# sisl/Crux.jl

Hardware: AMD Instinct MI355X
Metric: env-steps/sec + grad-steps/sec, PPO 2048x32 rollout (higher is better)
Workload: dtype f32

## Files before the change

### crux.jl_amd/csrc/train_fs2.hip

```cpp
#include "train_fs2_kernel.h"

template <int IN, int OUT, int KIND, int ACT, int H2, int ACT2, bool TIMING, bool PX = false, bool PXK = false, bool LAG = false>
static int32_t launch_fs2_form(crux_ctx* c, TrainArgs& a, hipStream_t stream) {
  using Lt = Fs2LayoutFor<IN, OUT, H2, LAG, PX>;
  constexpr size_t lds = sizeof(float) * (size_t)(PX && Lt::BK_FITS ? Lt::TOTAL_BK : Lt::TOTAL);
  { const int32_t rc = crux_lds_attr_once<k_train_fs2<IN, OUT, KIND, ACT, H2, ACT2, TIMING, PX, PXK, LAG>>(c, lds); if (rc) return rc; }
  hipLaunchKernelGGL((k_train_fs2<IN, OUT, KIND, ACT, H2, ACT2, TIMING, PX, PXK, LAG>), dim3(32), dim3(512), lds, stream, a);
  return crux_launch_check(c, PXK ? "k_train_fs2 (replica group, periodic form)" : PX ? "k_train_fs2 (replica group)" : LAG ? "k_train_fs2 (lagrange_ppo_loss)" : "k_train_fs2");
}
template <int IN, int OUT, int KIND, int ACT, int H2, int ACT2, unsigned FORMS>
static int32_t launch_fs2_row(crux_ctx* c, TrainArgs a, hipStream_t stream) {
  const int which = stream == c->stream ? 0 : 1;
  constexpr size_t xfloats = (size_t)CRUX_XBUF_FLOATS;
  if (!c->xbuf[which]) { if (hipMalloc(&c->xbuf[which], sizeof(float) * xfloats + 256) != hipSuccess) return crux_fail(c, CRUX_ENOMEM, "learner exchange buffer"); }
  a.xbuf = (float*)c->xbuf[which]; a.xctr = (unsigned*)((char*)c->xbuf[which] + sizeof(float) * xfloats);
  HIPCHK(c, hipMemsetAsync(c->xbuf[which], 0, sizeof(float) * xfloats + 256, stream));
  a.xcd = which;
  if constexpr ((FORMS & LF_FS2_LAG) != 0) { if (a.lag) return launch_fs2_form<IN, OUT, KIND, ACT, H2, ACT2, false, false, false, true>(c, a, stream); }
  if (crux_grouped(c) && a.need_px) {
    a.px_hist = c->peer_hist ? 1 : 0; a.px_n = c->peer_n; a.px_rank = c->peer_rank; a.px_tab = c->peer_tab + which * CRUX_PX_MAXR;
    if (a.px_every > 1) return launch_fs2_form<IN, OUT, KIND, ACT, H2, ACT2, false, true, true>(c, a, stream);
    return launch_fs2_form<IN, OUT, KIND, ACT, H2, ACT2, false, true, false>(c, a, stream);
  }
  if constexpr ((FORMS & LF_FS2_TIMING) != 0) if (crux_sw().mfma_timing) {
    a.dbg = mf_timing_buf(c);
    if (!a.dbg) return crux_fail(c, CRUX_ENOMEM, "timing buffer");
    int32_t rc = launch_fs2_form<IN, OUT, KIND, ACT, H2, ACT2, true>(c, a, stream); if (rc) return rc;
    static const char* const nc[16] = {"loop", "wait staged", "fwdL1+T1", "fwdL2", "L3+pair barrier+head", "dW3+dZ2+stats+T2", "wait B_1", "dW2+send+dH1", "dZ1+db+dW1", "B_2+reduce+granules", "wait P1",
                                       "W2 loads+granule poll", "drain loads", "totals+adam W2+ssq", "adam small", "B_b+report+exit"};
    static const char* const nh[16] = {"loop", "fetch", "stage next", "wait B_1", "dW2+send+drain", "arrival 1+wait(leader)", "-", "-", "-", "wait B_2+reduce+granules", "wait P1",
                                       "W2 loads+granule poll", "drain loads", "totals+adam W2+ssq", "adam small", "B_b+exit"};
    MfTimingRow rows[12];
    for (int i = 0; i < 12; ++i) { const int wg = i / 3, w = i % 3 == 0 ? 0 : i % 3 == 1 ? 4 : 7; rows[i].row = 8 * wg + w; rows[i].names = w == 0 ? nc : nh;
      snprintf(rows[i].label, sizeof rows[i].label, "[fs2-timing] %d-%d wg %d %s wave %d:", IN, OUT, wg, w == 0 ? "compute" : "helper", w); }
    return mf_timing_dump(c, stream, rows, 12);
  }
  return launch_fs2_form<IN, OUT, KIND, ACT, H2, ACT2, false>(c, a, stream);
}

int32_t crux_launch_fs2(crux_ctx* c, const TrainArgs& a, const LearnerShape* row, hipStream_t stream) {
#define FS2_ROW(I, O, K, A1, H, A2, F) if constexpr (((F) & LF_FS2_BUILT) != 0) if (row->is(I, O, K, A1, H, A2)) return launch_fs2_row<I, O, K, A1, H, A2, (F)>(c, a, stream);
  CRUX_LEARNER_SHAPES(FS2_ROW)
#undef FS2_ROW
  return crux_fail(c, CRUX_EINVAL, "k_train_fs2: no instantiation for this shape");
}
```

### crux.jl_amd/csrc/train_fs2_kernel.h

```cpp
#pragma once
#include <type_traits>
#include "train_args.h"

#include "mfma_helpers.h"
#include "learner_shared.h"
#include "peer_wait.h"

#define FS_LD 72
#ifndef CRUX_FS2_LATE_PARTS
#define CRUX_FS2_LATE_PARTS 3
#endif
__device__ __forceinline__ int fs_tx(int q) { return (4 - q) & 3; }

template <int IN, int OUT, int NWG, bool HELP = false, int H2 = 64, bool LAG = false>
struct FsLayout {
  static_assert(H2 == 64 || H2 == 32, "second hidden layer: 64 or 32 units");
  static constexpr int MH = H2 / 32, NT2 = H2 / 16, HH = H2 / 2, W2N = H2 * MF_HID;
  static constexpr int NWC = 16 / NWG, TILES = NWC / 2;
  static constexpr int NW = HELP ? 2 * NWC : NWC, NT = 64 * NW;
  static constexpr int NXB = HELP ? 2 : 1;
  static constexpr int KS0 = (IN + 3) / 4, IP = KS0 * 4, JT = (IN + 15) / 16, XP = IP + 2, W1LD = IP + 2;
  static constexpr int SCW = ((4 + (OUT > 4 ? OUT : 4)) | 1) + (LAG ? 2 : 0);
  static constexpr int ZW = OUT;
  static constexpr int sW1 = 0, sB1 = MF_HID * IN, sB2 = sB1 + MF_HID, sW3 = sB2 + H2, sB3 = sW3 + H2 * OUT, sEX = sB3 + OUT, NS = sEX + 16;
  static constexpr int cW1 = 0, cB1 = MF_HID * IN, cW2 = cB1 + MF_HID, cB2 = cW2 + W2N, cW3 = cB2 + H2, cB3 = cW3 + H2 * OUT, cEX = cB3 + OUT;
  static constexpr int W1ROWS = IP < 16 * JT ? IP : 16 * JT;
  static constexpr int pW1 = 0, pB1 = pW1 + W1ROWS * FS_LD, pB2 = pB1 + MF_HID, pW3 = pB2 + H2, pMISC = pW3 + OUT * H2;
  static constexpr int pST = pMISC, pB3 = pMISC + 7, pEX = pB3 + OUT;
  static constexpr int PART = ((pMISC + 48 + 3) / 4) * 4;
  static constexpr int NSP = ((NS + 3) / 4) * 4;
  static constexpr int TILE = MF_HID * 16, TILE2 = H2 * 16;
  static constexpr int oW2R = 0, oW2C = oW2R + H2 * FS_LD, oW1R = oW2C + MF_HID * FS_LD;
  static constexpr int oB1 = oW1R + MF_HID * W1LD, oB2 = oB1 + MF_HID, oW3R = oB2 + H2, oB3 = oW3R + OUT * H2, oEX = oB3 + 16;
  static constexpr int oMS = ((oEX + 16 + 3) / 4) * 4, oVS = oMS + NSP;
  static constexpr int oT1 = oVS + NSP, oT2 = oT1 + TILES * TILE;
  static constexpr int oD2X = oT2 + TILES * TILE2;
  static constexpr int oZP = oD2X + TILES * 2 * MH * 256;
  static constexpr int oPART = ((oZP + TILES * 2 * 64 * ZW + 3) / 4) * 4;
  static constexpr int oXS = oPART + TILES * PART;
  static constexpr int oSC = oXS + NXB * TILES * 16 * XP;
  static constexpr int oRED = oSC + NXB * TILES * 16 * SCW;
  static constexpr int oLAG = oRED + 32;
  static constexpr int oLGS = oLAG + (LAG ? 2 * 256 : 0);
  static constexpr int TOTAL = oLGS + (LAG ? 8 * NW : 0);
  static constexpr int NSI = (NS + NT - 1) / NT;
  static constexpr int XSLOT = ((W2N + NSI * NT + 16 + 3) / 4) * 4;
  static_assert(TOTAL <= 40960, "LDS budget (160 KB) exceeded");
  static_assert(XSLOT <= 8192, "exchange slot");
};

template <int IN, int OUT, int H2, bool LAG = false, bool MISC = false>
struct Fs2Layout : FsLayout<IN, OUT, 4, true, H2, LAG> {
  using B = FsLayout<IN, OUT, 4, true, H2, LAG>;
  static constexpr int NTC = 256;
  static constexpr bool MISC_MAP = MISC;
  static constexpr int NSD = MISC ? B::sB3 : B::NS;
  static constexpr int NSC = (NSD + 511) / 512;
  static constexpr int LB = MISC ? ((B::sB3 - 7) & 511) : 512 - 8;
  static constexpr int WT2 = (B::NT2 * 4) / 8;
  static constexpr int gST = NSC * 512;
  static constexpr int NGR = gST + (MISC ? 24 : 8);
  static constexpr int xW2 = 0, xGR = B::W2N;
  static constexpr int XSLOT2 = ((xGR + 2 * NGR + 3) / 4) * 4;
  static_assert(2 * 4 * XSLOT2 <= CRUX_XBUF_FLOATS, "exchange area");
  static constexpr bool BK_FITS = B::TOTAL + 3 * B::W2N <= 40960;
  static constexpr int oBK = B::TOTAL, TOTAL_BK = B::TOTAL + 3 * B::W2N;
  static constexpr int cACK = B::oRED + 18, cPAIR = B::oRED + 24, cCOMP = B::oRED + 26, fP1 = B::oRED + 29, fSUS = B::oRED + 30, fERR = B::oRED + 31;
  static constexpr int iLOSS = B::oRED + 19, iGN = B::oRED + 20, iENT = B::oRED + 21, iCLIP = B::oRED + 22, iADV = B::oRED + 23, iRET = B::oRED + 27;
  static constexpr int iPEN = B::oLGS + 5, iCUR = B::oLGS + 6, iCLOSS = B::oLGS + 7, iPLOSS = B::oLGS + 15;
};

template <int IN, int OUT, int H2, bool LAG> constexpr bool FS2_MISC_PAYS = Fs2Layout<IN, OUT, H2, LAG, true>::NSC < Fs2Layout<IN, OUT, H2, LAG, false>::NSC;
template <int IN, int OUT, int H2, bool LAG, bool PX> using Fs2LayoutFor = Fs2Layout<IN, OUT, H2, LAG, !PX && FS2_MISC_PAYS<IN, OUT, H2, LAG>>;

__device__ __forceinline__ void fs2_group_barrier(float* word, unsigned target, int lane) {
  unsigned* cnt = (unsigned*)word;
  asm volatile("s_waitcnt lgkmcnt(0)" ::: "memory");
  if (lane == 0) (void)__hip_atomic_fetch_add(cnt, 1u, __ATOMIC_RELAXED, __HIP_MEMORY_SCOPE_WORKGROUP);
  while (__hip_atomic_load(cnt, __ATOMIC_RELAXED, __HIP_MEMORY_SCOPE_WORKGROUP) < target) __builtin_amdgcn_s_sleep(0);
  asm volatile("" ::: "memory");
}
__device__ __forceinline__ void fs2_flag_set(float* word, unsigned v) { __hip_atomic_store((unsigned*)word, v, __ATOMIC_RELAXED, __HIP_MEMORY_SCOPE_WORKGROUP); }
__device__ __forceinline__ unsigned fs2_flag_get(const float* word) { return __hip_atomic_load((const unsigned*)word, __ATOMIC_RELAXED, __HIP_MEMORY_SCOPE_WORKGROUP); }
__device__ __forceinline__ void fs2_flag_wait(const float* word, unsigned target) {
  while (fs2_flag_get(word) < target) __builtin_amdgcn_s_sleep(0);
  asm volatile("" ::: "memory");
}

template <int IN, int OUT, int KIND, int ACT, int H2 = 64, int ACT2 = ACT, bool TIMING = false, bool PX = false, bool PXK = false, bool LAG = false>
__global__ __launch_bounds__(512) void k_train_fs2(TrainArgs a) {
  static_assert(!PXK || PX, "PXK: the periodic form of the replica group");
  static_assert(!LAG || (!PX && KIND != MFK_VALUE), "lagrange_ppo_loss: policy heads, one replica");
  static_assert(!PX || FsLayout<IN, OUT, 4, true, H2, false>::W2N + Fs2Layout<IN, OUT, H2, false, false>::NSC * 512 + 8 <= CRUX_PX_SEC, "a payload section must fit CRUX_PX_SEC");
  using Lt = Fs2LayoutFor<IN, OUT, H2, LAG, PX>;
  constexpr bool MISC = Lt::MISC_MAP;
  constexpr int NWG = 4, NWC = 4, TILES = 2, NT = 512, NTC = 256, MH = Lt::MH, HH = Lt::HH, W2N = Lt::W2N, NW = 8;
  constexpr int WT = Lt::WT2;
  constexpr int KS0 = Lt::KS0, IP = Lt::IP, JT = Lt::JT, XP = Lt::XP, NS = Lt::NS, NSC = Lt::NSC, XSLOT = Lt::XSLOT2;
  constexpr int NACT = (OUT > 4 ? OUT : 4);
  constexpr bool BK_LDS = PX && Lt::BK_FITS;
  if ((int)(blockIdx.x & 7) != a.xcd) return;
  constexpr bool PT = PXK && IN >= 27 && KIND == MFK_GAUSSIAN;
  constexpr bool PLAIN = !PX && !LAG;
  constexpr int NGW = OUT + (KIND == MFK_GAUSSIAN ? OUT : 0);
  constexpr bool STAT_SKIP = PLAIN && NGW <= 4 && !(TIMING && KIND == MFK_VALUE) && !(IN == 8 && OUT == 2 && KIND == MFK_GAUSSIAN);
  constexpr bool W2_TILED = PLAIN && WT == 2;
  constexpr int W3_PASSES = (OUT + 16 / (4 * MH) - 1) / (16 / (4 * MH));
  constexpr bool LATE_B2 = PLAIN && (CRUX_FS2_LATE_PARTS & 1) && W3_PASSES == 1;
  constexpr bool LATE_W3 = PLAIN && (CRUX_FS2_LATE_PARTS & 2);
  auto ka = [&]() { auto* q = (const __attribute__((address_space(4))) TrainArgs*)__builtin_amdgcn_kernarg_segment_ptr(); if constexpr (!PT) asm volatile("" : "+s"(q)); return q; };
  const int p = (int)(blockIdx.x >> 3);
  extern __shared__ __attribute__((aligned(16))) float sm[];
  typedef __attribute__((address_space(3))) float lds_f32;
  lds_f32* red3 = (lds_f32*)(sm + Lt::oRED); if constexpr (!PT) asm volatile("" : "+s"(red3));
  float* const smr = (float*)red3 - Lt::oRED;
  const int tid = threadIdx.x, lane = tid & 63, w = tid >> 6, c = lane & 15, g = lane >> 4;
  const bool cw = w < NWC;
  const int wt = w & (NWC - 1);
  const int t = wt >> 1, h = wt & 1;
  const int ct = tid & (NTC - 1);
  float* part = sm + Lt::oPART + t * Lt::PART;
  float* xs = sm + Lt::oXS + t * 16 * XP;
  float* sc = sm + Lt::oSC + t * 16 * Lt::SCW;
  constexpr int XSB = TILES * 16 * XP, SCB = TILES * 16 * Lt::SCW;
  int xcur = 0;
  float* T1 = sm + Lt::oT1 + t * Lt::TILE;
  float* T2 = sm + Lt::oT2 + t * Lt::TILE2;
  constexpr int n_extra = (KIND == MFK_GAUSSIAN) ? OUT : 0;
  unsigned long long tacc[16]; unsigned long long tlast = 0;
  if (TIMING) { for (int k = 0; k < 16; ++k) { tacc[k] = 0; asm volatile("" : "+v"(tacc[k])); } tlast = __builtin_amdgcn_s_memtime(); }
#define FS2_T(ph) do { if (TIMING) { const unsigned long long tn = __builtin_amdgcn_s_memtime(); tacc[ph] += tn - tlast; tlast = tn; } } while (0)
  const int t_wr = (4 * g) * 16 + 4 * ((c >> 2) ^ fs_tx(g)) + (c & 3);
  const int t_rd = c * 16 + 4 * (g ^ fs_tx(c >> 2));
  const int mp0 = (w * WT) >> 2, m0 = (w * WT) & 3;

  auto s_master = [](int s) { return slot_master<Lt, OUT, H2>(s); };
  auto s_canon = [](int s) { return slot_canon<Lt>(s); };
  auto s_part = [](int s) { return slot_part<Lt, OUT, H2, FS_LD>(s); };
  constexpr int ns_valid = Lt::sEX + n_extra, ns_dealt = MISC ? Lt::sB3 : ns_valid;

  for (int q = tid; q < W2N; q += NT) { const int o = q % H2, i = q / H2; const float v = a.p[Lt::cW2 + q];
    sm[Lt::oW2R + o * FS_LD + i] = v; sm[Lt::oW2C + i * FS_LD + o] = v; }
  for (int q = tid; q < MF_HID * Lt::W1LD; q += NT) sm[Lt::oW1R + q] = 0.f;
  if (tid < 16) { sm[Lt::oB3 + tid] = 0.f; sm[Lt::oEX + tid] = 0.f; }
  if (tid < 32) smr[Lt::oRED + tid] = 0.f;
  for (int q = tid; q < TILES * Lt::PART; q += NT) sm[Lt::oPART + q] = 0.f;
  uint32_t my_xcc = 0;
  if (tid == 0) { asm volatile("s_getreg_b32 %0, hwreg(HW_REG_XCC_ID)" : "=s"(my_xcc)); my_xcc &= 0xf;
    __hip_atomic_store(a.xctr + 8 + p, my_xcc + 1u, __ATOMIC_RELAXED, __HIP_MEMORY_SCOPE_AGENT); }
  __syncthreads();
  for (int s = tid; s < NS; s += NT) { const bool in = s < ns_valid; const int pc = s_canon(s);
    if (in) sm[s_master(s)] = a.p[pc];
    sm[Lt::oMS + s] = in ? a.m[pc] : 0.f; sm[Lt::oVS + s] = in ? a.v[pc] : 0.f; }
  for (int q = tid; q < Lt::NXB * TILES * 16 * XP; q += NT) sm[Lt::oXS + q] = 0.f;
  double bp1 = a.bp[0], bp2 = a.bp[1];
  const float lo = 1.f - a.eps_clip, hi = 1.f + a.eps_clip;
  const bool a2c = a.loss == CRUX_LOSS_A2C;
  AdamK ak; ak.b1 = (float)a.b1; ak.b2 = (float)a.b2; ak.omb1 = (float)(1.0 - a.b1); ak.omb2 = (float)(1.0 - a.b2); ak.eps = (float)a.eps; ak.eta = (float)a.eta;
  const double db1 = a.b1, db2 = a.b2;
  const float lambda_p = a.lambda_p, lambda_e = a.lambda_e, target_kl = a.target_kl, squash = a.squash;
  int kl_word = 0; if constexpr (!PT) { kl_word = __builtin_amdgcn_readfirstlane((KIND != MFK_VALUE && target_kl >= 0.f) ? 1 : 0); asm volatile("" : "+s"(kl_word)); }
  auto kl_on = [&]() -> bool { if constexpr (KIND == MFK_VALUE) return false; else if constexpr (PT) return target_kl >= 0.f; else return kl_word != 0; };
  const float kl_thr = PT ? 0.f : __builtin_bit_cast(float, __builtin_amdgcn_readfirstlane(__builtin_bit_cast(int, (KIND != MFK_VALUE && target_kl >= 0.f) ? target_kl : INFINITY)));
  auto kl_over = [&](float x) -> bool { if constexpr (KIND == MFK_VALUE) return false; else if constexpr (PT) return target_kl >= 0.f && x > target_kl; else return x > kl_thr; };
  auto is_t0 = [&]() -> bool { int t_ = tid; if constexpr (!PT) asm volatile("" : "+v"(t_)); return t_ == 0; };
  float pen = 0.f;
  float* lgs = sm + Lt::oLGS + 8 * w;
  if constexpr (LAG) { if (lane == 0) { lgs[0] = a.lag->I; lgs[1] = a.lag->smooth_delta; lgs[2] = a.lag->smooth_Jc; lgs[3] = a.lag->Jc_prev; lgs[4] = a.lag->deriv_term; lgs[5] = a.lag->penalty; lgs[6] = a.lag->cur_cost; lgs[7] = 0.f; } }
  auto lag_advance = [&](int buf) {
    const float* lc = sm + Lt::oLAG + 256 * buf;
    double sc_ = (double)lc[lane] + (double)lc[lane + 64], ne_ = (double)lc[128 + lane] + (double)lc[128 + lane + 64];
#pragma unroll
    for (int o_ = 32; o_ >= 1; o_ >>= 1) { sc_ += __shfl_xor(sc_, o_, 64); ne_ += __shfl_xor(ne_, o_, 64); }
    const crux_lagrange* L = a.lag;
    const float Jc = (float)sc_ / (float)ne_;
    const float dl = Jc - L->target_cost;
    float I_ = lgs[0], sd_ = lgs[1], sj_ = lgs[2]; const float jp_ = lgs[3];
    { const float x = I_ + L->Ki * dl; I_ = x > L->Ki_max ? L->Ki_max : (x < 0.f ? 0.f : x); }
    sd_ = (float)(L->ema_alpha * (double)sd_ + (1.0 - L->ema_alpha) * (double)dl);
    sj_ = (float)(L->ema_alpha * (double)sj_ + (1.0 - L->ema_alpha) * (double)Jc);
    float dt_; { const float x = sj_ - jp_; dt_ = (x != x) ? x : (x > 0.f ? x : 0.f); }
    { const float x = (L->Kp * sd_ + I_) + L->Kd * dt_; pen = x > L->penalty_max ? L->penalty_max : (x < 0.f ? 0.f : x); }
    if (lane == 0) { lgs[0] = I_; lgs[1] = sd_; lgs[2] = sj_; lgs[3] = sj_ ; lgs[4] = dt_; lgs[5] = pen; lgs[6] = Jc; }
  };
  const int max_batches = a.max_batches > 0 && a.max_batches < 0x7fffffffll ? (int)a.max_batches : 0;
  const int bs = a.bs;

  int32_t* order_cur = a.order_a; int32_t* order_nxt_pt = a.order_b;
  int total_batches = 0; int epochs_run = 0, err = 0, why_failed = 0; bool stop = false;
  bool staged = false;
  unsigned xstep = 0;
  float inf_kl = 0.f;
// ... 372 lines not shown
        adam_w2(gW2);
#pragma unroll
        for (int k = 0; k < NSC; ++k) bad_tot = bad_tot || (so_ok[k] && isnan(gs[k]));
        if (bad_tot) fs2_flag_set(smr + Lt::fSUS, tag);
      }
    } else if (!failed) {
      if constexpr (!W2_FIRST) { w2_total(gW2, pw); w2_check(gW2, want_ssq, ssq, bad_tot);
        adam_w2(gW2); }
#pragma unroll
      for (int k = 0; k < NSC; ++k) { gs[k] = (gs[k] + pg[0][k]) + (pg[1][k] + pg[2][k]); bad_tot = bad_tot || (so_ok[k] && isnan(gs[k])); }
      if constexpr (MISC) {
        stat_tot = (stat_loc + ps[0]) + (ps[1] + ps[2]);
        bad_tot = bad_tot || (own_lane && isnan(stat_tot));
        if (bad_tot) fs2_flag_set(smr + Lt::fSUS, tag);
      } else {
        if (bad_tot) fs2_flag_set(smr + Lt::fSUS, tag);
        stat_tot = (stat_loc + ps[0]) + (ps[1] + ps[2]);
      }
    }
    if (stat_lane && !own_lane) smr[Lt::oRED + 8 + (MISC && misc_k() > 7 ? 7 : misc_k())] = stat_tot;
#pragma unroll
    for (int k = 0; k < NSC; ++k) if (so_ok[k]) {
      if (!MISC && KIND == MFK_GAUSSIAN && so_ex[k]) gs[k] += LAG ? -lambda_e / (1.f + pen) : -lambda_e;
      if (want_ssq) ssq += gs[k] * gs[k]; }
    if constexpr (MISC) { if (own_lane) {
      if (KIND == MFK_GAUSSIAN && misc_k() >= 7 + OUT) stat_tot += LAG ? -lambda_e / (1.f + pen) : -lambda_e;
      if (want_ssq) ssq += stat_tot * stat_tot; } }
    if (want_ssq) { ssq = wave_sum(ssq);
      if (lane == 0) smr[Lt::oRED + w] = ssq; }
    FS2_T(13);
    auto adam_small = [&]() {
#pragma unroll
      for (int k = 0; k < NSC; ++k) { const int s = tid + NT * k;
        if (so_ok[k]) { float m_ = sm[Lt::oMS + s], v_ = sm[Lt::oVS + s]; const int mo = so_master[k]; const float th = sm[mo];
          m_o[k] = m_; v_o[k] = v_; th_o[k] = th;
          const float d = adam1(gs[k], m_, v_, ak);
          sm[Lt::oMS + s] = m_; sm[Lt::oVS + s] = v_; sm[mo] = th - d; } }
      if constexpr (MISC) { if (own_lane) { const int mi_s = Lt::sB3 + (misc_k() - 7), mi_master = s_master(mi_s);
          float m_ = sm[Lt::oMS + mi_s], v_ = sm[Lt::oVS + mi_s]; const float th = sm[mi_master];
          m_mo = m_; v_mo = v_; th_mo = th;
          const float d = adam1(stat_tot, m_, v_, ak);
          sm[Lt::oMS + mi_s] = m_; sm[Lt::oVS + mi_s] = v_; sm[mi_master] = th - d; } } };
    if (!failed) adam_small();
    if constexpr (PX && PXK) {
      if ((total_batches + 1) % a.px_every == 0) {
        float sT[NSC], sM[NSC], sV[NSC]; float dummy = 0.f;
#pragma unroll
        for (int k = 0; k < NSC; ++k) { const int s = tid + NT * k; const bool ok_ = so_ok[k] && !failed;
          sT[k] = ok_ ? sm[so_master[k]] : 0.f; sM[k] = ok_ ? sm[Lt::oMS + s] : 0.f; sV[k] = ok_ ? sm[Lt::oVS + s] : 0.f; }
        f32x4* const Wp[3] = {tW2, mW2, vW2}; float* const Sp[3] = {sT, sM, sV};
        const int rc = px_allreduce_mean(std::integral_constant<int, 3>{}, Wp, Sp, dummy, failed, tag, true);
        if (rc == 1) failed = true;
        if (rc == 0) {
#pragma unroll
          for (int k = 0; k < NSC; ++k) { const int s = tid + NT * k;
            if (so_ok[k]) { sm[so_master[k]] = sT[k]; sm[Lt::oMS + s] = sM[k]; sm[Lt::oVS + s] = sV[k]; } }
#pragma unroll
          for (int mm = 0; mm < WT; ++mm) {
#pragma unroll
            for (int r = 0; r < 4; ++r) sm[Lt::oW2R + (16 * mp0 + 4 * g + r) * FS_LD + 16 * (m0 + mm) + c] = tW2[mm][r];
            *(f32x4*)&sm[Lt::oW2C + (16 * (m0 + mm) + c) * FS_LD + 16 * mp0 + 4 * g] = tW2[mm]; } }
      }
    }
    FS2_T(14);
    __syncthreads();
    const unsigned why = fs2_flag_get(smr + Lt::fERR), sus = fs2_flag_get(smr + Lt::fSUS);
    if (why != 0u) { err = CRUX_EHIP; why_failed = (int)why; return false; }
    any_bad = 0;
    if (sus == tag) {
#pragma unroll
      for (int k = 0; k < NSC; ++k) { const int s = tid + NT * k;
        if (so_ok[k]) { sm[Lt::oMS + s] = m_o[k]; sm[Lt::oVS + s] = v_o[k]; sm[so_master[k]] = th_o[k]; } }
      if constexpr (MISC) { if (own_lane) { const int mi_s = Lt::sB3 + (misc_k() - 7), mi_master = s_master(mi_s);
          sm[Lt::oMS + mi_s] = m_mo; sm[Lt::oVS + mi_s] = v_mo; sm[mi_master] = th_mo; } }
#pragma unroll
      for (int mm = 0; mm < WT; ++mm) {
        if constexpr (BK_LDS) { tW2[mm] = *(const f32x4*)&bk[4 * NT * mm]; mW2[mm] = *(const f32x4*)&bk[4 * NT * (WT + mm)]; vW2[mm] = *(const f32x4*)&bk[4 * NT * (2 * WT + mm)]; }
        else { tW2[mm] = tW2o[mm]; mW2[mm] = mW2o[mm]; vW2[mm] = vW2o[mm]; } }
      any_bad = 1;
    }
    return true;
  };

  if (cw) {
    for (int ep = 0; ep < n_epochs && !stop && !err; ++ep) {
      if (!epoch_prologue(ep)) break;
      staged = false;
      for (int st = 0; st < total_rows; st += bs) {
        const int nb = (int)((total_rows - st) < bs ? (total_rows - st) : bs);
        const float invB = 1.0f / (float)nb;
        ak.c1 = __builtin_amdgcn_rcpf((float)(1.0 - bp1)); ak.c2 = __builtin_amdgcn_rcpf((float)(1.0 - bp2));
        FS2_T(0);
        if (!staged) __syncthreads();
        staged = false;
        if constexpr (LAG) lag_advance(xcur);
        const float* xs_c = xs + xcur * XSB; const float* sc_c = sc + xcur * SCB;
        FS2_T(1);
        auto want_stats = [&]() -> bool { return !STAT_SKIP || static_report(st) || kl_on() || epochs_run == 0; };
        f32x4 h1[4]; f32x4 h2[MH];
        f32x4 h2a[MH];
        constexpr bool W3_REG = OUT <= 2;
        f32x4 w3[OUT <= 2 ? OUT : 1][MH];
        float zp[OUT];
        {
          float xB[KS0];
#pragma unroll
          for (int ks = 0; ks < KS0; ++ks) xB[ks] = xs_c[c * XP + 4 * ks + g];
#pragma unroll
          for (int m = 0; m < 4; ++m) { f32x4 acc = *(const f32x4*)&sm[Lt::oB1 + 16 * m + 4 * g];
#pragma unroll
            for (int ks = 0; ks < KS0; ++ks) acc = __builtin_amdgcn_mfma_f32_16x16x4f32(sm[Lt::oW1R + (16 * m + c) * Lt::W1LD + 4 * ks + g], xB[ks], acc, 0, 0, 0);
#pragma unroll
            for (int r = 0; r < 4; ++r) acc[r] = actf<ACT>(acc[r]);
            h1[m] = acc; }
#pragma unroll
          for (int mm = 0; mm < 2; ++mm)
#pragma unroll
            for (int r = 0; r < 4; ++r) T1[t_wr + (16 * (2 * h + mm) + r) * 16] = (h ? (mm ? h1[3][r] : h1[2][r]) : (mm ? h1[1][r] : h1[0][r]));
          FS2_T(2);
          { f32x4 acc[MH];
#pragma unroll
            for (int mm = 0; mm < MH; ++mm) acc[mm] = *(const f32x4*)&sm[Lt::oB2 + HH * h + 16 * mm + 4 * g];
#pragma unroll
            for (int m = 0; m < 4; ++m) { f32x4 wv[MH];
#pragma unroll
              for (int mm = 0; mm < MH; ++mm) wv[mm] = *(const f32x4*)&sm[Lt::oW2R + (HH * h + 16 * mm + c) * FS_LD + 16 * m + 4 * g];
#pragma unroll
              for (int r = 0; r < 4; ++r)
#pragma unroll
                for (int mm = 0; mm < MH; ++mm) acc[mm] = __builtin_amdgcn_mfma_f32_16x16x4f32(wv[mm][r], h1[m][r], acc[mm], 0, 0, 0); }
#pragma unroll
            for (int mm = 0; mm < MH; ++mm) {
#pragma unroll
              for (int r = 0; r < 4; ++r) acc[mm][r] = actf<ACT2>(acc[mm][r]);
              h2[mm] = acc[mm]; } }
          FS2_T(3);
          if (W3_REG) {
#pragma unroll
            for (int o = 0; o < OUT; ++o)
#pragma unroll
              for (int mm = 0; mm < MH; ++mm) w3[o][mm] = *(const f32x4*)&sm[Lt::oW3R + o * H2 + HH * h + 16 * mm + 4 * g]; }
#pragma unroll
          for (int o = 0; o < OUT; ++o) { float acc = 0.f;
#pragma unroll
            for (int mm = 0; mm < MH; ++mm) { const f32x4 wv = W3_REG ? w3[W3_REG ? o : 0][mm] : *(const f32x4*)&sm[Lt::oW3R + o * H2 + HH * h + 16 * mm + 4 * g];
#pragma unroll
              for (int r = 0; r < 4; ++r) acc = fmaf(wv[r], h2[mm][r], acc); }
            zp[o] = g4_sum(acc); }
          { float* zq = sm + Lt::oZP + ((t * 2 + h) * 64 + lane) * Lt::ZW;
#pragma unroll
            for (int o = 0; o < OUT; ++o) zq[o] = zp[o]; }
        }
        fs2_group_barrier(smr + Lt::cPAIR + t, 2u * (xstep + 1u), lane);
        float dz[OUT], dex[OUT];
        float s_lossp = 0.f, s_H = 0.f, s_kl = 0.f, s_adv = 0.f, s_ret = 0.f, s_clip = 0.f, s_sq = 0.f, s_cost = 0.f;
        float ent_pre = 1.4189385332046727f;
        {
          float z[OUT];
          { const float* zo = sm + Lt::oZP + ((t * 2 + (1 - h)) * 64 + lane) * Lt::ZW;
#pragma unroll
            for (int o = 0; o < OUT; ++o) { const float other = zo[o]; z[o] = (h ? other + zp[o] : zp[o] + other) + sm[Lt::oB3 + o]; } }
          {
            const float* q = sc_c + c * Lt::SCW;
            const bool valid = q[0] != 0.f; const float oldlp = q[1], A = q[2], R = q[3];
            const float cnt = (valid && g == 0) ? 1.f : 0.f;
#pragma unroll
// ... 32 lines not shown
                inr[k] = (sq && !(ls >= -5.f && ls <= 2.f)) ? 0.f : 1.f;
                newlp += (-(dd[k] * dd[k]) * (0.5f * s2[k]) - 0.9189385332046727f - ls); }
              if (squash > 0.f) newlp -= q[4 + NACT];
              const float r = __expf(newlp - oldlp); const float u = r * A, rc = fminf(fmaxf(r, lo), hi), cl = rc * A; const float gsel = (u <= cl) ? A : 0.f;
              const float coef = a2c ? A : gsel * r, lterm = a2c ? newlp * A : fminf(u, cl), clipv = (!a2c && (r > hi || r < lo)) ? 1.f : 0.f;
              float cf = -lambda_p * coef;
              if constexpr (LAG) { const float Ac = q[Lt::SCW - 1]; const float uc = r * Ac, clc = rc * Ac; s_cost = cnt * (uc >= clc ? uc : clc);
                cf = (cf + pen * ((uc >= clc ? Ac : 0.f) * r)) / (1.f + pen); }
#pragma unroll
              for (int k = 0; k < OUT; ++k) { dz[k] = valid ? invB * (cf * (dd[k] * s2[k])) : 0.f;
                dex[k] = valid ? invB * (cf * (((dd[k] * dd[k]) * s2[k]) * inr[k] - 1.f)) : 0.f; }
              s_lossp = cnt * lterm; s_kl = cnt * (oldlp - newlp); s_adv = cnt * A; s_ret = cnt * R; s_clip = cnt * clipv;
            }
          }
          FS2_T(4);
          if (KIND == MFK_GAUSSIAN) {
#pragma unroll
            for (int k = 0; k < OUT; ++k) ent_pre += sm[Lt::oEX + k]; }
          constexpr int FPL = 4 * MH, PER = 16 / FPL;
#define FS2_DW3_PART(HV) \
          _Pragma("unroll") \
          for (int o2 = 0; o2 < (OUT + PER - 1) / PER; ++o2) { float pv[16]; \
            _Pragma("unroll") \
            for (int oo = 0; oo < PER; ++oo) \
              _Pragma("unroll") \
              for (int mm = 0; mm < MH; ++mm) \
                _Pragma("unroll") \
                for (int r = 0; r < 4; ++r) pv[FPL * oo + 4 * mm + r] = (PER * o2 + oo < OUT) ? dz[(PER * o2 + oo < OUT) ? PER * o2 + oo : 0] * HV[mm][r] : 0.f; \
            const float sred = row16_reduce_scatter(pv, c); \
            const int oo = c / FPL; \
            if (PER * o2 + oo < OUT) part[Lt::pW3 + (PER * o2 + oo) * H2 + HH * h + 16 * ((c >> 2) & (MH - 1)) + 4 * g + (c & 3)] = sred; }
          if constexpr (LATE_W3) {
#pragma unroll
            for (int mm = 0; mm < MH; ++mm) h2a[mm] = h2[mm];
          } else { FS2_DW3_PART(h2) }
          { f32x4 d2[MH];
#pragma unroll
            for (int mm = 0; mm < MH; ++mm) d2[mm] = (f32x4){0.f, 0.f, 0.f, 0.f};
#pragma unroll
            for (int o = 0; o < OUT; ++o)
#pragma unroll
              for (int mm = 0; mm < MH; ++mm) { const f32x4 wv = W3_REG ? w3[W3_REG ? o : 0][mm] : *(const f32x4*)&sm[Lt::oW3R + o * H2 + HH * h + 16 * mm + 4 * g];
#pragma unroll
                for (int r = 0; r < 4; ++r) d2[mm][r] = fmaf(wv[r], dz[o], d2[mm][r]); }
#pragma unroll
            for (int mm = 0; mm < MH; ++mm)
#pragma unroll
              for (int r = 0; r < 4; ++r) h2[mm][r] = actg<ACT2>(h2[mm][r], d2[mm][r]); }
          if (STAT_SKIP && h == 0 && !want_stats()) {
            float gq = 0.f;
            int ln = lane; asm volatile("" : "+v"(ln));
#pragma unroll
            for (int o = 0; o < NGW; ++o) { const float tot = row16_sum_all(o < OUT ? dz[o < OUT ? o : 0] : dex[o < OUT ? 0 : o - OUT]); gq = ((ln & 15) == 7 + o) ? tot : gq; }
            if ((unsigned)(ln - 7) < (unsigned)NGW) part[Lt::pMISC + ln] = gq;
          } else
          if (h == 0) {
            constexpr int NVB = 7 + OUT + (KIND == MFK_GAUSSIAN ? OUT : 0), NV = NVB + (LAG ? 1 : 0);
            float mv[((NV + 15) / 16) * 16];
#pragma unroll
            for (int k = 0; k < ((NV + 15) / 16) * 16; ++k) mv[k] = 0.f;
            mv[0] = s_lossp; mv[1] = s_H; mv[2] = s_kl; mv[3] = s_adv; mv[4] = s_ret; mv[5] = s_clip; mv[6] = s_sq;
#pragma unroll
            for (int o = 0; o < OUT; ++o) { mv[7 + o] = dz[o]; if (KIND == MFK_GAUSSIAN) mv[7 + OUT + o] = dex[o]; }
            if constexpr (LAG) mv[NVB] = s_cost;
#pragma unroll
            for (int ch = 0; ch < (NV + 15) / 16; ++ch) { float cv[16];
#pragma unroll
              for (int k = 0; k < 16; ++k) cv[k] = mv[16 * ch + k];
              const float tq = row16_reduce_scatter(cv, c);
              if (g == 0) part[Lt::pMISC + 16 * ch + c] = tq; } }
#pragma unroll
          for (int mm = 0; mm < MH; ++mm)
#pragma unroll
            for (int r = 0; r < 4; ++r) T2[t_wr + (16 * (MH * h + mm) + r) * 16] = h2[mm][r];
          { float* dq = sm + Lt::oD2X + ((t * 2 + h) * MH) * 256 + lane * 4;
#pragma unroll
            for (int mm = 0; mm < MH; ++mm) *(f32x4*)&dq[256 * mm] = h2[mm]; }
        }
        FS2_T(5);
        __syncthreads();
        FS2_T(6);
        f32x4 gW2[WT];
        dw2_send(gW2);
        if constexpr (LATE_B2) {
          float gb2[MH];
#pragma unroll
          for (int mm = 0; mm < MH; ++mm) { float sb2 = 0.f;
            const f32x4 d2 = *(const f32x4*)&T2[t_rd + 256 * (MH * h + mm)];
#pragma unroll
            for (int r = 0; r < 4; ++r) sb2 += d2[r];
            gb2[mm] = g4_sum(sb2); }
          if (g == 0) {
#pragma unroll
            for (int mm = 0; mm < MH; ++mm) part[Lt::pB2 + HH * h + 16 * mm + c] = gb2[mm]; } }
        f32x4 dz1r[2];
        { const float* dq = sm + Lt::oD2X + ((t * 2 + (1 - h)) * MH) * 256 + lane * 4;
          f32x4 av[2 * MH];
#pragma unroll
          for (int mm = 0; mm < MH; ++mm) { av[mm] = h2[mm]; av[MH + mm] = *(const f32x4*)&dq[256 * mm]; }
          f32x4 acc0 = {0.f, 0.f, 0.f, 0.f}, acc1 = {0.f, 0.f, 0.f, 0.f};
#pragma unroll
          for (int q = 0; q < 2 * MH; ++q) { const int fo = HH * ((q >= MH) ? 1 - h : h) + 16 * (q % MH);
            const f32x4 wv0 = *(const f32x4*)&sm[Lt::oW2C + (32 * h + c) * FS_LD + fo + 4 * g];
            const f32x4 wv1 = *(const f32x4*)&sm[Lt::oW2C + (32 * h + 16 + c) * FS_LD + fo + 4 * g];
#pragma unroll
            for (int r = 0; r < 4; ++r) { acc0 = __builtin_amdgcn_mfma_f32_16x16x4f32(av[q][r], wv0[r], acc0, 0, 0, 0);
              acc1 = __builtin_amdgcn_mfma_f32_16x16x4f32(av[q][r], wv1[r], acc1, 0, 0, 0); } }
          dz1r[0] = acc0; dz1r[1] = acc1; }
        asm volatile("s_waitcnt vmcnt(0)" ::: "memory");
        if (lane == 0) (void)__hip_atomic_fetch_add((unsigned*)(smr + Lt::cACK), 1u, __ATOMIC_RELAXED, __HIP_MEMORY_SCOPE_WORKGROUP);
        FS2_T(7);
        if constexpr (LATE_W3) { constexpr int FPL = 4 * MH, PER = 16 / FPL; FS2_DW3_PART(h2a) }
#undef FS2_DW3_PART
        float gb1[2], gb2[MH];
#pragma unroll
        for (int mm = 0; mm < 2; ++mm) { float sb1 = 0.f;
          const f32x4 h1r = *(const f32x4*)&T1[t_rd + 256 * (2 * h + mm)];
#pragma unroll
          for (int r = 0; r < 4; ++r) { const float d = actg<ACT>(h1r[r], dz1r[mm][r]); dz1r[mm][r] = d; sb1 += d; }
          gb1[mm] = g4_sum(sb1); }
        if constexpr (!LATE_B2) {
#pragma unroll
        for (int mm = 0; mm < MH; ++mm) { float sb2 = 0.f;
          const f32x4 d2 = *(const f32x4*)&T2[t_rd + 256 * (MH * h + mm)];
#pragma unroll
          for (int r = 0; r < 4; ++r) sb2 += d2[r];
          gb2[mm] = g4_sum(sb2); } }
        if (g == 0) {
#pragma unroll
          for (int mm = 0; mm < 2; ++mm) part[Lt::pB1 + 32 * h + 16 * mm + c] = gb1[mm];
          if constexpr (!LATE_B2) {
#pragma unroll
          for (int mm = 0; mm < MH; ++mm) part[Lt::pB2 + HH * h + 16 * mm + c] = gb2[mm]; } }
#pragma unroll
        for (int jt = 0; jt < JT; ++jt) {
          float xR[4];
#pragma unroll
          for (int r = 0; r < 4; ++r) xR[r] = (16 * jt + c < IP) ? xs_c[(4 * g + r) * XP + 16 * jt + c] : 0.f;
#pragma unroll
          for (int mm = 0; mm < 2; ++mm) { f32x4 acc = {0.f, 0.f, 0.f, 0.f};
#pragma unroll
            for (int r = 0; r < 4; ++r) acc = __builtin_amdgcn_mfma_f32_16x16x4f32(dz1r[mm][r], xR[r], acc, 0, 0, 0);
            if (16 * jt + c < Lt::W1ROWS) *(f32x4*)&part[Lt::pW1 + (16 * jt + c) * FS_LD + 32 * h + 16 * mm + 4 * g] = acc; }
        }
        FS2_T(8);
        fs2_group_barrier(smr + Lt::cCOMP, (unsigned)NWC * (xstep + 1u), lane);
        const unsigned tag = xstep + 1u;
        int any_bad = 0; st_now = st;
        if (!step_tail(tag, gW2, any_bad)) break;
        if (any_bad || static_report(st) || kl_on()) {
          const float* tq = smr + Lt::oRED + 8;
          const bool report = any_bad || static_report(st) || kl_over(tq[2] * invB);
          if (report) {
            float ss = smr[Lt::oRED];
#pragma unroll
            for (int q = 1; q < NW; ++q) ss += smr[Lt::oRED + q];
            if (KIND != MFK_VALUE) inf_kl = tq[2] * invB;
            if (is_t0()) { smr[Lt::iGN] = sqrtf(ss);
              if (KIND == MFK_VALUE) { smr[Lt::iLOSS] = tq[6] * invB; smr[Lt::iRET] = tq[4] * invB; }
              else { const float p_loss = -(tq[0] * invB); const float entropy = KIND == MFK_CATEGORICAL ? tq[1] * invB : ent_pre;
                smr[Lt::iENT] = entropy; smr[Lt::iLOSS] = fmaf(lambda_p, p_loss, lambda_e * (-entropy)); smr[Lt::iADV] = tq[3] * invB; smr[Lt::iRET] = tq[4] * invB; smr[Lt::iCLIP] = tq[5] * invB;
                if constexpr (LAG) { const float cost_loss = pen * (tq[7] * invB);
                  smr[Lt::iLOSS] = ((lambda_p * p_loss + lambda_e * (-entropy)) + cost_loss) / (1.f + pen);
                  smr[Lt::iCLOSS] = cost_loss; smr[Lt::iPLOSS] = lambda_p * p_loss; } } } } }
        const bool go = step_exit(invB, any_bad != 0);
        if (!any_bad) { bp1 *= db1; bp2 *= db2; }
        xcur ^= 1; xstep += 1u; staged = st + bs < total_rows;
        FS2_T(15);
        if (!go) break;
      }
      if (err) break;
      epoch_epilogue(ep);
    }
  } else {
    constexpr int NXL = (IN + 3) / 4;
    float px[NXL]; float p_lp = 0.f, p_adv = 0.f, p_ret = 0.f; float p_act[NACT]; int p_valid = 0; uint8_t p_abyte[OUT];
#pragma unroll
    for (int k = 0; k < OUT; ++k) p_abyte[k] = 0;
#pragma unroll
    for (int k = 0; k < NACT; ++k) p_act[k] = 0.f;
#pragma unroll
    for (int e = 0; e < NXL; ++e) px[e] = 0.f;
    int n_row = 0, n_valid = 0;
    int n_row2 = -1; float p_cost2 = 0.f, p_ee2 = 0.f, p_cadv = 0.f;
    constexpr bool PK_V = !PT && !(PXK && IN >= 24 && KIND == MFK_GAUSSIAN);
    const float* pk_base = a.PACK; int pk_stride = a.pack_stride, pk_lp = a.pack_lp, pk_act = a.pack_act;
    if constexpr (PK_V) asm volatile("" : "+v"(pk_base), "+v"(pk_stride), "+v"(pk_lp), "+v"(pk_act));
    int pk_word = 0; if constexpr (!PT) { pk_word = __builtin_amdgcn_readfirstlane(a.PACK ? 1 : 0); asm volatile("" : "+s"(pk_word)); }
    auto packed = [&]() -> bool { if constexpr (PT) return a.PACK != nullptr; else return pk_word != 0; };
    auto fetch_index = [&](const int32_t* ord, int st, int nb) {
      const int sidx = 8 * NWC * p + 16 * t + c;
      n_valid = sidx < nb ? 1 : 0;
      n_row = n_valid ? CRUX_GLOBAL_PTR(int32_t, ord)[st + sidx] : 0;
      if constexpr (LAG) n_row2 = ct < nb ? CRUX_GLOBAL_PTR(int32_t, ord)[st + ct] : -1;
    };
    auto fetch_data = [&]() {
      int h = wt & 1, lane = tid & 63; if constexpr (!PT) asm volatile("" : "+v"(h), "+v"(lane));
      const int rowlo = n_row; p_valid = n_valid; const int64_t row = rowlo;
      if constexpr (LAG) { const auto* k = ka(); p_cost2 = n_row2 >= 0 ? CRUX_GLOBAL_PTR(float, k->COST)[n_row2] : 0.f; p_ee2 = (n_row2 >= 0 && CRUX_GLOBAL_PTR(uint8_t, k->EE)[n_row2]) ? 1.f : 0.f; }
      if (h == 0) {
        const int rs = __shfl(rowlo, lane >> 2, 64), vs = __shfl(p_valid, lane >> 2, 64);
        const float* xrow = packed() ? CRUX_GLOBAL_PTR(float, pk_base) + (int64_t)rs * pk_stride + (lane & 3) * NXL : CRUX_GLOBAL_PTR(float, ka()->S) + (int64_t)rs * IN + (lane & 3) * NXL;
#pragma unroll
        for (int e = 0; e < NXL; ++e) px[e] = ((lane & 3) * NXL + e < IN && vs) ? xrow[e] : 0.f;
      } else {
        p_lp = 0.f; p_adv = 0.f; p_ret = 0.f; p_cadv = 0.f;
#pragma unroll
        for (int k = 0; k < NACT; ++k) p_act[k] = 0.f;
        if (packed() && !LAG) {
          if (lane < 16 && p_valid) { const float* q = CRUX_GLOBAL_PTR(float, pk_base) + row * pk_stride;
            if (KIND != MFK_VALUE) { p_lp = q[pk_lp]; p_adv = q[pk_lp + 1]; }
            p_ret = q[pk_lp + 2];
            if (KIND == MFK_CATEGORICAL) { const int ai = (int)q[pk_act];
#pragma unroll
              for (int k = 0; k < OUT; ++k) p_abyte[k] = k == ai ? 1 : 0; }
            if (KIND == MFK_GAUSSIAN) {
#pragma unroll
              for (int k = 0; k < OUT; ++k) p_act[k] = q[pk_act + k]; } }
        } else
        if (lane < 16 && p_valid) { const auto* k = ka();
          if constexpr (LAG) p_cadv = CRUX_GLOBAL_PTR(float, k->CADV)[row];
          if (KIND != MFK_VALUE) { p_lp = CRUX_GLOBAL_PTR(float, k->LP)[row]; p_adv = CRUX_GLOBAL_PTR(float, k->ADV)[row]; }
          { const float* const RET = k->RET; p_ret = RET ? CRUX_GLOBAL_PTR(float, RET)[row] : 0.f; }
          if (KIND == MFK_CATEGORICAL) { const auto* av = CRUX_GLOBAL_PTR(uint8_t, k->A) + row * OUT;
#pragma unroll
            for (int k = 0; k < OUT; ++k) p_abyte[k] = av[k]; }
          if (KIND == MFK_GAUSSIAN) { const auto* av = CRUX_GLOBAL_PTR(float, k->A) + row * OUT;
#pragma unroll
            for (int k = 0; k < OUT; ++k) p_act[k] = av[k]; }
        }
      }
    };
    auto stage = [&](int buf) {
      float* xs_ = xs + buf * XSB; float* sc_ = sc + buf * SCB;
      if constexpr (LAG) { if (ct < 128) { sm[Lt::oLAG + 256 * buf + ct] = p_cost2; sm[Lt::oLAG + 256 * buf + 128 + ct] = p_ee2; } }
      if (h == 0) {
#pragma unroll
        for (int e = 0; e < NXL; ++e) { const int f = (lane & 3) * NXL + e; if (f < IN) xs_[(lane >> 2) * XP + f] = px[e]; }
      } else {
        if (KIND == MFK_CATEGORICAL) { int ai = 0;
#pragma unroll
          for (int k = 0; k < OUT; ++k) ai = p_abyte[k] ? k : ai;
          p_act[0] = (float)ai; }
        if (lane < 16) { float* q = sc_ + lane * Lt::SCW; q[0] = (float)p_valid; q[1] = p_lp; q[2] = p_adv; q[3] = p_ret;
          if constexpr (LAG) q[Lt::SCW - 1] = p_cadv;
          if (KIND == MFK_GAUSSIAN) {
            static_assert(KIND != MFK_GAUSSIAN || ((4 + NACT) % 2 == 0), "the staging row needs its spare slot");
            float corr = 0.f;
            if (squash > 0.f) {
#pragma unroll
              for (int k = 0; k < OUT; ++k) { const float u = p_valid ? sq_untanh(p_act[k], squash) : 0.f; corr += p_valid ? sq_corr(u) : 0.f; p_act[k] = u; } }
            q[4 + NACT] = corr; }
#pragma unroll
          for (int k = 0; k < NACT; ++k) q[4 + k] = p_act[k]; }
      }
    };

    for (int ep = 0; ep < n_epochs && !stop && !err; ++ep) {
      if (!epoch_prologue(ep)) break;
      staged = false;
      { const int nb0 = (int)(total_rows < bs ? total_rows : bs); fetch_index(order_cur, 0, nb0); fetch_data();
        const int st1 = bs; const int nb1 = st1 < total_rows ? (int)((total_rows - st1) < bs ? (total_rows - st1) : bs) : 0; fetch_index(order_cur, st1 < total_rows ? st1 : 0, nb1); }
      for (int st = 0; st < total_rows; st += bs) {
        const int nb = (int)((total_rows - st) < bs ? (total_rows - st) : bs);
        const float invB = 1.0f / (float)nb;
        ak.c1 = __builtin_amdgcn_rcpf((float)(1.0 - bp1)); ak.c2 = __builtin_amdgcn_rcpf((float)(1.0 - bp2));
        FS2_T(0);
        if (!staged) { stage(xcur); __syncthreads(); }
        staged = false;
        if constexpr (LAG) lag_advance(xcur);
        if (st + bs < total_rows) fetch_data();
        { const int st2 = st + 2 * bs; const int nb2 = st2 < total_rows ? (int)((total_rows - st2) < bs ? (total_rows - st2) : bs) : 0;
          fetch_index(order_cur, st2 < total_rows ? st2 : 0, nb2); }
        FS2_T(1);
        if (st + bs < total_rows) stage(xcur ^ 1);
        FS2_T(2);
        __syncthreads();
        FS2_T(3);
        const unsigned tag = xstep + 1u;
        f32x4 gW2[WT];
        dw2_send(gW2);
        asm volatile("s_waitcnt vmcnt(0)" ::: "memory");
        if (lane == 0) (void)__hip_atomic_fetch_add((unsigned*)(smr + Lt::cACK), 1u, __ATOMIC_RELAXED, __HIP_MEMORY_SCOPE_WORKGROUP);
        FS2_T(4);
        if (ct == 0) {
          fs2_flag_wait(smr + Lt::cACK, (unsigned)NW * tag);
          (void)__hip_atomic_fetch_add(a.xctr + 4, 1u, __ATOMIC_RELAXED, __HIP_MEMORY_SCOPE_AGENT);
          const unsigned want = (unsigned)NWG * tag; unsigned spins = 0; bool ok = true;
          while (__hip_atomic_load(a.xctr + 4, __ATOMIC_RELAXED, __HIP_MEMORY_SCOPE_AGENT) < want) { __builtin_amdgcn_s_sleep(1);
            if (++spins > (1u << 24) || __hip_atomic_load(a.xctr + 1, __ATOMIC_RELAXED, __HIP_MEMORY_SCOPE_AGENT) != 0u) { ok = false; break; } }
          unsigned why = ok ? 0u : 1u;
          if (ok && xstep == 0u) {
            uint32_t xcc = 0; asm volatile("s_getreg_b32 %0, hwreg(HW_REG_XCC_ID)" : "=s"(xcc)); xcc &= 0xf;
            for (int q = 0; q < NWG; ++q) { const unsigned peer_xcc = __hip_atomic_load(a.xctr + 8 + q, __ATOMIC_RELAXED, __HIP_MEMORY_SCOPE_AGENT);
              if (peer_xcc != xcc + 1u) { ok = false; why = 2u; } } }
          if (!ok) { __hip_atomic_store(a.xctr + 1, 1u, __ATOMIC_RELAXED, __HIP_MEMORY_SCOPE_AGENT); if (fs2_flag_get(smr + Lt::fERR) == 0u) fs2_flag_set(smr + Lt::fERR, why); }
          fs2_flag_set(smr + Lt::fP1, tag);
        }
        FS2_T(5);
        fs2_flag_wait(smr + Lt::cCOMP, (unsigned)NWC * tag);
        int any_bad = 0; st_now = st;
        if (!step_tail(tag, gW2, any_bad)) break;
        const bool go = step_exit(invB, any_bad != 0);
        if (!any_bad) { bp1 *= db1; bp2 *= db2; }
        xcur ^= 1; xstep += 1u; staged = st + bs < total_rows;
        FS2_T(15);
        if (!go) break;
      }
      if (err) break;
      epoch_epilogue(ep);
    }
  }
  __syncthreads();
  const auto* kz = ka(); float* const P = kz->p; float* const M = kz->m; float* const V = kz->v;
  if (p == 0) {
    int tid2 = tid; asm volatile("" : "+v"(tid2));
    const int lane2 = tid2 & 63, w2_ = tid2 >> 6, c2 = lane2 & 15, g2 = lane2 >> 4, mp2 = (w2_ * WT) >> 2, m2 = (w2_ * WT) & 3;
#pragma unroll
    for (int mm = 0; mm < WT; ++mm)
#pragma unroll
      for (int r = 0; r < 4; ++r) { const int pc = Lt::cW2 + (16 * mp2 + 4 * g2 + r) + H2 * (16 * (m2 + mm) + c2);
        P[pc] = tW2[mm][r]; M[pc] = mW2[mm][r]; V[pc] = vW2[mm][r]; } }
  if (p == 0) { for (int s = tid; s < ns_valid; s += NT) { const int pc = s_canon(s); P[pc] = sm[s_master(s)]; M[pc] = sm[Lt::oMS + s]; V[pc] = sm[Lt::oVS + s]; } }
  if (TIMING && lane == 0) { if (unsigned long long* const dbg = kz->dbg) { for (int k = 0; k < 16; ++k) dbg[(NW * p + w) * 16 + k] = tacc[k]; } }
  if (PX && tid == 0 && p == 0) *(unsigned long long*)(px_mine + CRUX_PX_COUNT) = px0 + (unsigned long long)pxc;
  if constexpr (PX && PXK) {
    if (tid == 0 && p == 0 && err == CRUX_ENAN) { for (int r = 0; r < kz->px_n; ++r) if (r != kz->px_rank) __hip_atomic_store((unsigned*)(kz->px_tab[r] + CRUX_PX_ABORT), 5u, __ATOMIC_RELAXED, __HIP_MEMORY_SCOPE_SYSTEM); } }
  if (tid == 0 && (p == 0 || err)) { int32_t* const status = kz->status; double* const bp = kz->bp; float* const infos = kz->epoch_infos;
    status[0] = err; status[1] = (int32_t)total_batches; status[2] = epochs_run; status[3] = (order_cur == kz->order_a) ? 0 : 1;
    if (err == CRUX_EHIP) status[4] = why_failed;
    bp[0] = bp1; bp[1] = bp2;
    if constexpr (LAG) { if (p == 0) { crux_lagrange* const lag = kz->lag; lag->I = lgs[0]; lag->smooth_delta = lgs[1]; lag->smooth_Jc = lgs[2]; lag->Jc_prev = lgs[3]; lag->deriv_term = lgs[4]; lag->penalty = lgs[5]; lag->cur_cost = lgs[6]; } }
    if (err && infos && epochs_run == 0) { infos[CRUX_INFO_LOSS] = smr[Lt::iLOSS]; infos[CRUX_INFO_GRAD_NORM] = NAN; }
  }
#undef FS2_T
}
```

Baseline: 315,100.

## Move db2 reduction to helper waves and post LDS ack mid-dH1 MFMA loop

Compute waves now post their cACK arrival partway through the dH1 MFMA loop (after ACK_K of the K-steps), not after it finishes, so helpers can start the cross-workgroup arrival sooner. The db2 partial reduction moves off the compute waves into the helper waves, which then join the cCOMP barrier (B2_WAVES doubles to NW). The aim is to shorten the compute waves' critical path before the group barrier and overlap the inter-XCD arrival with the remaining MFMA work. The cost is more complex synchronisation with new counts, and a risk of ordering bugs if the W2 staging is not complete at the early ack point.

```diff
diff --git a/crux.jl_amd/csrc/train_fs2.hip b/crux.jl_amd/csrc/train_fs2.hip
--- a/crux.jl_amd/csrc/train_fs2.hip
+++ b/crux.jl_amd/csrc/train_fs2.hip
@@ -28,7 +28,7 @@
     int32_t rc = launch_fs2_form<IN, OUT, KIND, ACT, H2, ACT2, true>(c, a, stream); if (rc) return rc;
     static const char* const nc[16] = {"loop", "wait staged", "fwdL1+T1", "fwdL2", "L3+pair barrier+head", "dW3+dZ2+stats+T2", "wait B_1", "dW2+send+dH1", "dZ1+db+dW1", "B_2+reduce+granules", "wait P1",
                                        "W2 loads+granule poll", "drain loads", "totals+adam W2+ssq", "adam small", "B_b+report+exit"};
-    static const char* const nh[16] = {"loop", "fetch", "stage next", "wait B_1", "dW2+send+drain", "arrival 1+wait(leader)", "-", "-", "-", "wait B_2+reduce+granules", "wait P1",
+    static const char* const nh[16] = {"loop", "fetch", "stage next", "wait B_1", "dW2+send+drain", "arrival 1+wait(leader)", "acks+arrival 1 (HELP_B2)", "db2 (HELP_B2)", "-", "wait B_2+reduce+granules", "wait P1",
                                        "W2 loads+granule poll", "drain loads", "totals+adam W2+ssq", "adam small", "B_b+exit"};
     MfTimingRow rows[12];
     for (int i = 0; i < 12; ++i) { const int wg = i / 3, w = i % 3 == 0 ? 0 : i % 3 == 1 ? 4 : 7; rows[i].row = 8 * wg + w; rows[i].names = w == 0 ? nc : nh;
diff --git a/crux.jl_amd/csrc/train_fs2_kernel.h b/crux.jl_amd/csrc/train_fs2_kernel.h
--- a/crux.jl_amd/csrc/train_fs2_kernel.h
+++ b/crux.jl_amd/csrc/train_fs2_kernel.h
@@ -9,6 +9,15 @@
 #define FS_LD 72
 #ifndef CRUX_FS2_LATE_PARTS
 #define CRUX_FS2_LATE_PARTS 3
+#endif
+#ifndef CRUX_FS2_ACK_K
+#define CRUX_FS2_ACK_K 4
+#endif
+#ifndef CRUX_FS2_HELPER_PARTS
+#define CRUX_FS2_HELPER_PARTS 1
+#endif
+#ifndef CRUX_FS2_HELP_TIMERS
+#define CRUX_FS2_HELP_TIMERS 0
 #endif
 __device__ __forceinline__ int fs_tx(int q) { return (4 - q) & 3; }
 
@@ -108,6 +117,11 @@
   constexpr int W3_PASSES = (OUT + 16 / (4 * MH) - 1) / (16 / (4 * MH));
   constexpr bool LATE_B2 = PLAIN && (CRUX_FS2_LATE_PARTS & 1) && W3_PASSES == 1;
   constexpr bool LATE_W3 = PLAIN && (CRUX_FS2_LATE_PARTS & 2);
+  constexpr bool EA_FORM = PLAIN && !(KIND == MFK_VALUE && (IN == 27 || (IN == 17 && H2 == 32)));
+  constexpr int DH1_KS = 8 * MH, ACK_KS = EA_FORM && (CRUX_FS2_ACK_K) < 16 ? ((CRUX_FS2_ACK_K) * DH1_KS) / 16 : DH1_KS;
+  constexpr bool HELP_B2 = LATE_B2 && EA_FORM && ((CRUX_FS2_HELPER_PARTS) & 1);
+  constexpr bool EARLY_ACK = ACK_KS < DH1_KS && (HELP_B2 || !((CRUX_FS2_HELPER_PARTS) & 1));
+  constexpr int B2_WAVES = HELP_B2 ? NW : NWC;
   auto ka = [&]() { auto* q = (const __attribute__((address_space(4))) TrainArgs*)__builtin_amdgcn_kernarg_segment_ptr(); if constexpr (!PT) asm volatile("" : "+s"(q)); return q; };
   const int p = (int)(blockIdx.x >> 3);
   extern __shared__ __attribute__((aligned(16))) float sm[];
@@ -646,6 +660,17 @@
     return true;
   };
 
+#define FS2_DB2_PART \
+        { float gb2[MH]; \
+          _Pragma("unroll") \
+          for (int mm = 0; mm < MH; ++mm) { float sb2 = 0.f; \
+            const f32x4 d2 = *(const f32x4*)&T2[t_rd + 256 * (MH * h + mm)]; \
+            _Pragma("unroll") \
+            for (int r = 0; r < 4; ++r) sb2 += d2[r]; \
+            gb2[mm] = g4_sum(sb2); } \
+          if (g == 0) { \
+            _Pragma("unroll") \
+            for (int mm = 0; mm < MH; ++mm) part[Lt::pB2 + HH * h + 16 * mm + c] = gb2[mm]; } }
   if (cw) {
     for (int ep = 0; ep < n_epochs && !stop && !err; ++ep) {
       if (!epoch_prologue(ep)) break;
@@ -844,18 +869,27 @@
         FS2_T(6);
         f32x4 gW2[WT];
         dw2_send(gW2);
-        if constexpr (LATE_B2) {
-          float gb2[MH];
-#pragma unroll
-          for (int mm = 0; mm < MH; ++mm) { float sb2 = 0.f;
-            const f32x4 d2 = *(const f32x4*)&T2[t_rd + 256 * (MH * h + mm)];
-#pragma unroll
-            for (int r = 0; r < 4; ++r) sb2 += d2[r];
-            gb2[mm] = g4_sum(sb2); }
-          if (g == 0) {
-#pragma unroll
-            for (int mm = 0; mm < MH; ++mm) part[Lt::pB2 + HH * h + 16 * mm + c] = gb2[mm]; } }
+        if constexpr (LATE_B2 && !HELP_B2) FS2_DB2_PART
         f32x4 dz1r[2];
+        if constexpr (EARLY_ACK) {
+          const float* dq = sm + Lt::oD2X + ((t * 2 + (1 - h)) * MH) * 256 + lane * 4;
+          f32x4 av[2 * MH], wv0[2 * MH], wv1[2 * MH];
+#pragma unroll
+          for (int mm = 0; mm < MH; ++mm) { av[mm] = h2[mm]; av[MH + mm] = *(const f32x4*)&dq[256 * mm]; }
+#pragma unroll
+          for (int q = 0; q < 2 * MH; ++q) { const int fo = HH * ((q >= MH) ? 1 - h : h) + 16 * (q % MH);
+            wv0[q] = *(const f32x4*)&sm[Lt::oW2C + (32 * h + c) * FS_LD + fo + 4 * g];
+            wv1[q] = *(const f32x4*)&sm[Lt::oW2C + (32 * h + 16 + c) * FS_LD + fo + 4 * g]; }
+          f32x4 acc0 = {0.f, 0.f, 0.f, 0.f}, acc1 = {0.f, 0.f, 0.f, 0.f};
+#pragma unroll
+          for (int ks = 0; ks < DH1_KS; ++ks) { const int q = ks >> 2, r = ks & 3;
+            if (ks == ACK_KS) {
+              asm volatile("s_waitcnt vmcnt(0)" : "+v"(acc0), "+v"(acc1) :: "memory");
+              if (lane == 0) (void)__hip_atomic_fetch_add((unsigned*)(smr + Lt::cACK), 1u, __ATOMIC_RELAXED, __HIP_MEMORY_SCOPE_WORKGROUP); }
+            acc0 = __builtin_amdgcn_mfma_f32_16x16x4f32(av[q][r], wv0[q][r], acc0, 0, 0, 0);
+            acc1 = __builtin_amdgcn_mfma_f32_16x16x4f32(av[q][r], wv1[q][r], acc1, 0, 0, 0); }
+          dz1r[0] = acc0; dz1r[1] = acc1;
+        } else {
         { const float* dq = sm + Lt::oD2X + ((t * 2 + (1 - h)) * MH) * 256 + lane * 4;
           f32x4 av[2 * MH];
 #pragma unroll
@@ -871,6 +905,7 @@
           dz1r[0] = acc0; dz1r[1] = acc1; }
         asm volatile("s_waitcnt vmcnt(0)" ::: "memory");
         if (lane == 0) (void)__hip_atomic_fetch_add((unsigned*)(smr + Lt::cACK), 1u, __ATOMIC_RELAXED, __HIP_MEMORY_SCOPE_WORKGROUP);
+        }
         FS2_T(7);
         if constexpr (LATE_W3) { constexpr int FPL = 4 * MH, PER = 16 / FPL; FS2_DW3_PART(h2a) }
 #undef FS2_DW3_PART
@@ -906,7 +941,7 @@
             if (16 * jt + c < Lt::W1ROWS) *(f32x4*)&part[Lt::pW1 + (16 * jt + c) * FS_LD + 32 * h + 16 * mm + 4 * g] = acc; }
         }
         FS2_T(8);
-        fs2_group_barrier(smr + Lt::cCOMP, (unsigned)NWC * (xstep + 1u), lane);
+        fs2_group_barrier(smr + Lt::cCOMP, (unsigned)B2_WAVES * (xstep + 1u), lane);
         const unsigned tag = xstep + 1u;
         int any_bad = 0; st_now = st;
         if (!step_tail(tag, gW2, any_bad)) break;
@@ -1045,9 +1080,24 @@
         asm volatile("s_waitcnt vmcnt(0)" ::: "memory");
         if (lane == 0) (void)__hip_atomic_fetch_add((unsigned*)(smr + Lt::cACK), 1u, __ATOMIC_RELAXED, __HIP_MEMORY_SCOPE_WORKGROUP);
         FS2_T(4);
+        if constexpr (HELP_B2) {
+          if (ct == 0) {
+            fs2_flag_wait(smr + Lt::cACK, (unsigned)NW * tag);
+            (void)__hip_atomic_fetch_add(a.xctr + 4, 1u, __ATOMIC_RELAXED, __HIP_MEMORY_SCOPE_AGENT); }
+          if constexpr (CRUX_FS2_HELP_TIMERS) FS2_T(6);
+          {
+            int tl = tid; asm volatile("" : "+v"(tl));
+            const int c = tl & 15, g = (tl >> 4) & 3, h = (tl >> 6) & 1;
+            FS2_DB2_PART }
+          asm volatile("s_waitcnt lgkmcnt(0)" ::: "memory");
+          if (lane == 0) (void)__hip_atomic_fetch_add((unsigned*)(smr + Lt::cCOMP), 1u, __ATOMIC_RELAXED, __HIP_MEMORY_SCOPE_WORKGROUP);
+          if constexpr (CRUX_FS2_HELP_TIMERS) FS2_T(7);
+        }
         if (ct == 0) {
+          if constexpr (!HELP_B2) {
           fs2_flag_wait(smr + Lt::cACK, (unsigned)NW * tag);
           (void)__hip_atomic_fetch_add(a.xctr + 4, 1u, __ATOMIC_RELAXED, __HIP_MEMORY_SCOPE_AGENT);
+          }
           const unsigned want = (unsigned)NWG * tag; unsigned spins = 0; bool ok = true;
           while (__hip_atomic_load(a.xctr + 4, __ATOMIC_RELAXED, __HIP_MEMORY_SCOPE_AGENT) < want) { __builtin_amdgcn_s_sleep(1);
             if (++spins > (1u << 24) || __hip_atomic_load(a.xctr + 1, __ATOMIC_RELAXED, __HIP_MEMORY_SCOPE_AGENT) != 0u) { ok = false; break; } }
@@ -1060,7 +1110,7 @@
           fs2_flag_set(smr + Lt::fP1, tag);
         }
         FS2_T(5);
-        fs2_flag_wait(smr + Lt::cCOMP, (unsigned)NWC * tag);
+        fs2_flag_wait(smr + Lt::cCOMP, (unsigned)B2_WAVES * tag);
         int any_bad = 0; st_now = st;
         if (!step_tail(tag, gW2, any_bad)) break;
         const bool go = step_exit(invB, any_bad != 0);
@@ -1095,5 +1145,6 @@
     if constexpr (LAG) { if (p == 0) { crux_lagrange* const lag = kz->lag; lag->I = lgs[0]; lag->smooth_delta = lgs[1]; lag->smooth_Jc = lgs[2]; lag->Jc_prev = lgs[3]; lag->deriv_term = lgs[4]; lag->penalty = lgs[5]; lag->cur_cost = lgs[6]; } }
     if (err && infos && epochs_run == 0) { infos[CRUX_INFO_LOSS] = smr[Lt::iLOSS]; infos[CRUX_INFO_GRAD_NORM] = NAN; }
   }
+#undef FS2_DB2_PART
 #undef FS2_T
 }
```

New measurement: 321,800, median of 6. 1.02x the previous value.
